# mathwrx/Decouple-and-Couple_Learning_in_Multi-Modal_Brain_Tumor_Segmentation

Hardware: AMD Instinct MI355X
Metric: training volumes/sec (4x128^3) (higher is better)
Workload: dtype bf16x3 forward (split-bf16 MFMA operands hi.hi+hi.lo+lo.hi: logits within 1e-3 of the fp32 reference) / bf16 data-gradient / bf16 weight-gradient MFMA operands; f32 accumulate, f32 storage, f32 master weights; 1 GPU; configs[1]: 1xMI355X, batch 2 per GPU, 4-modality 128^3 synthetic BraTS patches; fwd + softmax_dice + 4 sub-region/edge losses + bwd + Adam(amsgrad); random-init weights, dropout on; global_batch=2, parallelism=dp1, precision=bf16x3, dgrad_precision=bf16, wgrad_precision=bf16, mode=plan

## Files before the change

decouple-and-couple_learning_in_multi-modal_brain_tumor_segmentation_amd/csrc/conv_args.h:

```cpp
#pragma once
#include "common.h"

typedef __bf16 bf16x8 __attribute__((ext_vector_type(8)));
typedef unsigned u32x4 __attribute__((ext_vector_type(4)));

struct ConvArgsB {
  ConvGeom g;
  const float* x; const uint4* wpk; const float* bias; float* y;
  const float* in_scale; const float* in_shift; float in_slope;
  const float* residual; int r_ldc; const float* out_scale; double* stats;
  unsigned long long unused_[2];
  const float* nb_x; int nb_ldc; const float* nb_scale; const float* nb_shift; float nb_slope;
  int groups, x_goff, y_goff;
  const uint4* wpk_g[3]; const float* bias_g[3];
  const uint4* x16; const uint4* zero16;
  unsigned short* y16;
};

typedef __bf16 bf16x2_t __attribute__((ext_vector_type(2)));
typedef float f32x2_t __attribute__((ext_vector_type(2)));
__device__ __forceinline__ unsigned pack_bf16(float a, float b) {
  const f32x2_t f = {a, b};
  return __builtin_bit_cast(unsigned, __builtin_convertvector(f, bf16x2_t));
}
__device__ __forceinline__ float bf16_round(float a) { return (float)(__bf16)a; }
__device__ __forceinline__ void split_bf16(float a, float b, unsigned& hi, unsigned& lo) {
  hi = pack_bf16(a, b);
  const float ha = __builtin_bit_cast(float, hi << 16), hb = __builtin_bit_cast(float, hi & 0xffff0000u);
  lo = pack_bf16(a - ha, b - hb);
}
__device__ __forceinline__ float act01(float v, float slope) { return fmaxf(v, v * slope); }


static inline int cfg_extent(int op, int Di, int Hi, int Wi, int Do, int Ho, int Wo, int cd[3]) {
  cd[0] = Do; cd[1] = Ho; cd[2] = Wo;
  if (op == CWF_CONVT2) { cd[0] = Di; cd[1] = Hi; cd[2] = Wi; return 8; }
  if (op == CWF_CONV3_S2_DGRAD) { cd[0] = (Do + 1) / 2; cd[1] = (Ho + 1) / 2; cd[2] = (Wo + 1) / 2; return 8; }
  return 1;
}

int cwf_try_conv_ws(int op, int x3, ConvArgsB& a, hipStream_t st, int* rc);
int cwf_ws_takes_x16(int op, int N, int D, int H, int W, int Cin, int Cout);
int cwf_ws_takes_x3();
int cwf_try_conv_wsp(int op, int x3, int cfg_mt, int cfg_wm, ConvArgsB& a, hipStream_t st, int* rc);
int cwf_try_conv_wsd(int op, int x3, int cfg_mt, int cfg_wm, ConvArgsB& a, hipStream_t st, int* rc);

int conv_fp32_launch(const cwf_conv_args& d, hipStream_t st);
int conv_stem_launch(const cwf_conv_args& d, hipStream_t st);
int conv_s2c16_launch(const cwf_conv_args& d, hipStream_t st);
int wgrad_fp32_launch(const cwf_wgrad_args& d, int* nsplit_used, hipStream_t st);
```

decouple-and-couple_learning_in_multi-modal_brain_tumor_segmentation_amd/csrc/conv_bf16.hip:

```cpp
#include "common.h"
#include <cstdio>
#include <cstdlib>
#include <type_traits>

#include "conv_args.h"

#define CB_MAXS 13
struct StageSlots { int goff[CB_MAXS]; unsigned inb; int nslots; };

__device__ __forceinline__ void stage_slots_init(StageSlots& ss, const ConvGeom& g, int id0, int ih0, int iw0, int tid) {
  const int nvox_in = g.ID * g.IH * g.IW;
  ss.nslots = (nvox_in + 63) >> 6; ss.inb = 0u;
  const int dq = 64 / g.IW, dr = 64 - dq * g.IW;
  int iw = (tid >> 2) % g.IW, t2 = (tid >> 2) / g.IW;
  int ih = t2 % g.IH, idd = t2 / g.IH;
#pragma unroll
  for (int i = 0; i < CB_MAXS; ++i) {
    const int v = (tid >> 2) + 64 * i;
    const int gd = id0 + idd, gh = ih0 + ih, gw = iw0 + iw;
    const bool ok = v < nvox_in && gd >= 0 && gd < g.Di && gh >= 0 && gh < g.Hi && gw >= 0 && gw < g.Wi;
    ss.goff[i] = ok ? ((gd * g.Hi + gh) * g.Wi + gw) * g.x_ldc : 0;
    ss.inb |= ok ? (1u << i) : 0u;
    iw += dr; int adv = dq;
    if (iw >= g.IW) { iw -= g.IW; ++adv; }
// ... 1149 lines not shown
    }
    if (d.y16) return CWF_E_BADARG;
  }
  {
    int rcw = 0;
    if (cwf_try_conv_wsp(op, x3, c.MT, c.WM, a, st, &rcw)) return rcw;
    if (cwf_try_conv_wsd(op, x3, c.MT, c.WM, a, st, &rcw)) return rcw;
    if (cwf_try_conv_ws(op, x3, a, st, &rcw)) return rcw;
  }
  if (op == CWF_CONV3_S1 && Cin <= 16 && Cout <= 16) c16_tap_order(a.g);
  if (op == CWF_CONV3_S1 && Cin <= 16 && Cout <= 16 && (int64_t)d.Do * d.Ho * d.Wo >= 32768) {
    rc = cwf_build_geom(a.g, op, N, d.Di, d.Hi, d.Wi, Cin, x_ldc, d.Do, d.Ho, d.Wo, Cout, y_ldc, 16);
    if (rc) return rc;
    return x3 ? launch_conv16s<true>(a, st) : launch_conv16s<false>(a, st);
  }
#define CWF_CFG(mt, nt, wm) if (c.MT == mt && c.NT == nt && c.WM == wm) return x3 ? launch_cfg<mt, nt, wm, true>(a, st) : launch_cfg<mt, nt, wm, false>(a, st);
  CWF_CFG(4, 4, 1) CWF_CFG(2, 4, 2) CWF_CFG(2, 4, 4) CWF_CFG(4, 2, 4) CWF_CFG(4, 1, 4)
  CWF_CFG(1, 4, 4) CWF_CFG(1, 2, 4) CWF_CFG(1, 2, 2) CWF_CFG(1, 1, 4)
#undef CWF_CFG
  return CWF_E_BADARG;
}

static int conv_grouped_impl(const cwf_conv_args& d, hipStream_t st) {
  const int op = d.op, x3 = d.precision == CWF_BF16X3, groups = d.groups, N = d.N, Cin = d.Cin, Cout = d.Cout;
  const int x_ldc = d.x_ldc, y_ldc = d.y_ldc, x_goff = d.x_goff, y_goff = d.y_goff;
  if (!d.x || !d.y || N <= 0 || Cin <= 0 || Cout <= 0) return CWF_E_BADARG;
  if ((Cin & 3) || (x_ldc & 3) || (x_goff & 3) || x_ldc < (groups - 1) * x_goff + Cin || y_ldc < (groups - 1) * y_goff + Cout) return CWF_E_ALIGN;
  if ((uintptr_t)d.x & 15) return CWF_E_ALIGN;
  ConvArgsB a;
  int cd[3];
  TileCfg c = choose_cfg(op, cd, cfg_extent(op, d.Di, d.Hi, d.Wi, d.Do, d.Ho, d.Wo, cd), N * groups, cdiv(Cout, 16));
  int rc = cwf_build_geom(a.g, op, N, d.Di, d.Hi, d.Wi, Cin, x_ldc, d.Do, d.Ho, d.Wo, Cout, y_ldc, c.MT * c.WM);
  if (rc) return rc;
  a.x = d.x; a.wpk = nullptr; a.bias = nullptr; a.y = d.y; a.in_scale = nullptr; a.in_shift = nullptr; a.in_slope = 1.f;
  a.residual = nullptr; a.r_ldc = 0; a.out_scale = nullptr; a.stats = nullptr;
  a.nb_x = nullptr; a.nb_ldc = 0; a.nb_scale = nullptr; a.nb_shift = nullptr; a.nb_slope = 1.f;
  a.groups = groups; a.x_goff = x_goff; a.y_goff = y_goff;
  a.x16 = nullptr; a.zero16 = nullptr; a.y16 = nullptr;
  for (int q = 0; q < 3; ++q) {
    a.wpk_g[q] = q < groups ? reinterpret_cast<const uint4*>(d.wpk_g[q]) : nullptr;
    a.bias_g[q] = q < groups ? d.bias_g[q] : nullptr;
    if (q < groups && (!d.wpk_g[q] || ((uintptr_t)d.wpk_g[q] & 15))) return CWF_E_ALIGN;
  }
  if (Cin <= 16 && Cout <= 16) c16_tap_order(a.g);
#define CWF_CFG(mt, nt, wm) if (c.MT == mt && c.NT == nt && c.WM == wm) return x3 ? launch_cfg<mt, nt, wm, true>(a, st) : launch_cfg<mt, nt, wm, false>(a, st);
  CWF_CFG(4, 4, 1) CWF_CFG(2, 4, 2) CWF_CFG(2, 4, 4) CWF_CFG(4, 2, 4) CWF_CFG(4, 1, 4)
  CWF_CFG(1, 4, 4) CWF_CFG(1, 2, 4) CWF_CFG(1, 2, 2) CWF_CFG(1, 1, 4)
#undef CWF_CFG
  return CWF_E_BADARG;
}

extern "C" int cwf_conv_x16_ok(int op, int N, int D, int H, int W, int Cin, int Cout) {
  if (op != CWF_CONV3_S1 || N <= 0 || D <= 0 || H <= 0 || W <= 0) return 0;
  if (Cin == 16 && Cout == 16) return (int64_t)D * H * W >= 32768 && (int64_t)N * D * H * W < (1ll << 30);
  return cwf_ws_takes_x16(op, N, D, H, W, Cin, Cout);
}

extern "C" int cwf_conv(const struct cwf_conv_args* args, void* stream) {
  if (!args) return CWF_E_BADARG;
  const cwf_conv_args& d = *args;
  if (d.precision != CWF_FP32 && d.precision != CWF_BF16X3 && d.precision != CWF_BF16) return CWF_E_BADARG;
  const bool fp32 = d.precision == CWF_FP32;
  hipStream_t st = cwf_stream(stream);
  if (d.groups) {
    if (d.groups < 2 || d.groups > 3 || d.op != CWF_CONV3_S1 || d.in_scale || d.residual || d.out_scale || d.stats || d.nb_x || d.x16 ||
        d.y16 || d.w_raw)
      return CWF_E_BADARG;
    if (!fp32) return conv_grouped_impl(d, st);
    for (int q = 0; q < d.groups; ++q) {
      cwf_conv_args g = d;
      g.groups = 0; g.x = d.x + q * d.x_goff; g.y = d.y + q * d.y_goff; g.wpk = d.wpk_g[q]; g.bias = d.bias_g[q];
      const int rc = conv_fp32_launch(g, st);
      if (rc) return rc;
    }
    return 0;
  }
  if (d.x16) {
    if (d.precision != CWF_BF16 || d.in_scale || d.out_scale || d.y16 || !d.zero16 || ((uintptr_t)d.x16 & 15) || ((uintptr_t)d.zero16 & 15))
      return CWF_E_BADARG;
    if (d.Do != d.Di || d.Ho != d.Hi || d.Wo != d.Wi || !cwf_conv_x16_ok(d.op, d.N, d.Di, d.Hi, d.Wi, d.Cin, d.Cout))
      return CWF_E_BADARG;
    return conv_bf16_impl(d, st);
  }
  if (d.y16) {
    if (d.nb_x || d.out_scale) return CWF_E_BADARG;
    if (!fp32 && d.op == CWF_CONV1) {
      const int rc = conv_bf16_impl(d, st);
      if (rc != CWF_E_BADARG) return rc;
    }
    cwf_conv_args f = d;
    f.y16 = nullptr;
    const int rc = cwf_conv(&f, stream);
    if (rc) return rc;
    return cwf_to_bf16(d.y, d.y_ldc, nullptr, nullptr, 1.f, d.y16, d.N, (int64_t)d.Do * d.Ho * d.Wo, d.Cout, stream);
  }
  const int64_t vo = (int64_t)d.Do * d.Ho * d.Wo;
  if (d.w_raw && !fp32 && !d.in_scale && !d.residual && !d.nb_x) {
    if (d.op == CWF_CONV3_S1 && d.Cin == 4 && d.Cout == 16 && vo >= 32768) return conv_stem_launch(d, st);
    if (d.op == CWF_CONV3_S2 && d.Cin == 16 && d.Cout == 32 && !d.out_scale && vo >= 32768 &&
        d.Do == (d.Di + 1) / 2 && d.Ho == (d.Hi + 1) / 2 && d.Wo == (d.Wi + 1) / 2)
      return conv_s2c16_launch(d, st);
  }
  if (fp32) return d.nb_x ? CWF_E_BADARG : conv_fp32_launch(d, st);
  return conv_bf16_impl(d, st);
}
```

decouple-and-couple_learning_in_multi-modal_brain_tumor_segmentation_amd/cwf/_lib.py:

```python
from __future__ import annotations

import ctypes as C
import os

_HERE = os.path.dirname(os.path.abspath(__file__))
LIB_PATH = os.path.join(_HERE, "libcwf_hip.so")

P = C.c_void_p
I = C.c_int
L = C.c_int64
F = C.c_float
U = C.c_uint32
U64 = C.c_uint64
D = C.c_double

SIGNATURES = {
    "cwf_version": [],
    "cwf_conv": [P, P],
    "cwf_conv_x16_ok": [I, I, I, I, I, I, I],
    "cwf_debug_wsd": [I],
    "cwf_debug_wsd_launches": [],
    "cwf_wgrad": [P, P, P],
    "cwf_debug_wgrad_bf16_plan": [P, P],
    "cwf_debug_wgrad_bf16_name": [I],
    "cwf_debug_wgrad_s2": [I],
    "cwf_debug_wgrad_s2_launches": [],
    "cwf_gather_split_bf16": [P, I, L, P],
    "cwf_wgrad_nsplit": [I, I, I, I, I, I, I],
    "cwf_wgrad_partial_floats": [I, I, I, I, I, I, I],
    "cwf_wgrad_slab_floats": [I, I, I],
    "cwf_wgrad_reduce": [P, I, L, P, P, P, P],
    "cwf_gather_batched": [P, I, L, P],
    "cwf_in_finalize": [P, P, P, I, L, F, P],
    "cwf_in_stats": [P, I, P, I, L, I, P],
    "cwf_norm_act_add": [P, I, P, P, F, P, I, P, I, I, L, I, P],
    "cwf_in_bwd_stats": [P, I, P, I, P, P, F, P, I, L, I, P],
    "cwf_in_bwd_apply": [P, I, P, I, P, P, F, P, P, I, P, I, I, L, I, P],
    "cwf_in_bwd_apply_ex": [P, I, P, I, P, P, F, P, P, I, P, I, P, P, I, L, I, P],
    "cwf_norm_act_add_ex": [P, I, P, P, F, P, I, P, I, P, I, L, I, P],
    "cwf_to_bf16": [P, I, P, P, F, P, I, L, I, P],
    "cwf_gemm": [P, L, L, L, L, P, L, L, L, L, P, L, L, L, P, P, L, L, L, I, I, I, I, I, F, I, I, P],
    "cwf_layernorm_fwd": [P, P, P, P, P, P, I, I, F, P],
    "cwf_layernorm_bwd": [P, P, P, P, P, P, P, P, I, I, I, P],
    "cwf_softmax_rows": [P, L, I, I, P],
    "cwf_softmax_rows_bwd": [P, P, L, I, I, P],
    "cwf_gelu_bwd": [P, P, P, L, P],
    "cwf_colsum": [P, L, I, I, P, I, P],
    "cwf_window_to_tokens": [P, I, P, I, I, I, I, I, I, I, I, P],
    "cwf_tokens_to_window": [P, P, I, I, I, I, I, I, I, I, I, I, P],
    "cwf_token_scores": [P, P, L, P, I, I, I, P],
    "cwf_topk": [P, P, I, I, I, P],
    "cwf_gather_tokens": [P, P, P, L, P, F, P, I, I, I, I, P],
    "cwf_gather_tokens_bwd": [P, P, P, P, P, L, I, I, I, I, P],
    "cwf_scatter_rows": [P, P, P, L, L, P, L, P, I, I, I, I, P],
    "cwf_scatter_rows_bwd": [P, P, P, P, L, P, I, P, L, L, P, L, I, I, I, I, P],
    "cwf_upsample_softmax": [P, I, P, I, I, I, I, I, I, P],
    "cwf_upsample_softmax_bwd": [P, P, P, I, I, I, I, I, I, I, P, P],
    "cwf_channel_softmax": [P, I, P, L, I, P],
    "cwf_channel_softmax_bwd": [P, P, P, I, L, I, P],
    "cwf_dice_ce_sums": [P, P, U, P, I, L, I, P],
    "cwf_dice_ce_finalize": [P, P, P, I, L, I, P],
    "cwf_dice_ce_bwd": [P, P, U, P, P, P, I, L, I, P],
    "cwf_adam_amsgrad": [P, I, L, C.c_double, C.c_double, C.c_double, C.c_double, C.c_double, I, I, P, P],
    "cwf_adam_amsgrad_scaled": [P, I, L, C.c_double, C.c_double, C.c_double, C.c_double, C.c_double, I, I, P, F, P],
    "cwf_grad_add": [P, P, P, L, P],
    "cwf_grad_norm_clip": [P, L, F, F, P, P, P],
    "cwf_adam_amsgrad_ex": [P, I, L, C.c_double, C.c_double, C.c_double, C.c_double, C.c_double, I, I, P, F, P, P, F, P],
    "cwf_optim_step": [I, P, I, L, C.c_double, C.c_double, P, C.c_double, C.c_double, C.c_double, I, I, P, C.c_double, C.c_double, I, I,
                       F, P, P, F, P],
    "cwf_wgrad_reduce_batched": [P, I, P],
    "cwf_dropout_mask": [P, L, F, F, C.c_uint64, C.c_uint64, P],
    "cwf_mul": [P, P, P, L, P],
    "cwf_add": [P, P, P, L, P],
    "cwf_channel_scale": [P, I, P, P, I, I, L, I, P],
    "cwf_copy_strided": [P, I, P, I, L, I, P],
    "cwf_add3": [P, P, P, P, L, P],
    "cwf_bcast3": [P, P, L, P],
    "cwf_stats_channel_sum": [P, P, I, I, P],
    "cwf_gemm_ex": [P, P],
    "cwf_debug_gemm_panel": [I],
    "cwf_debug_gemm_panel_launches": [],
    "cwf_attn_fwd": [P, L, P, L, I, I, I, I, F, P, U64, F, P],
    "cwf_attn_bwd": [P, L, P, L, P, I, I, I, I, F, P, U64, F, P],
    "cwf_attn_bwd_ws": [P, L, P, L, P, I, I, I, I, F, P, U64, F, P, L, P],
    "cwf_attn_bwd_ws_bytes": [I, I, I],
    "cwf_debug_attn_split": [I],
    "cwf_debug_attn_split_waves": [I],
    "cwf_debug_attn_split_launches": [],
    "cwf_ln_pair_fwd": [P, P, I, P, P, P, P, P, P, P, I, I, F, P],
    "cwf_ln_pair_bwd": [P, P, P, P, P, I, P, P, P, P, P, P, P, P, P, I, I, I, P],
    "cwf_gelu_bwd_drop": [P, P, P, L, P, U64, F, P],
    "cwf_token_scores2": [P, P, L, P, L, P, P, I, I, I, P],
    "cwf_topk_inv": [P, P, P, P, P, P, I, I, I, P],
    "cwf_index_inv": [P, P, I, I, I, P],
    "cwf_gather_multi": [P, I, I, I, I, F, P, F, P],
    "cwf_scatter_inv": [P, P, P, L, L, P, L, P, P, I, I, I, P],
    "cwf_scatter_bwd": [P, P, P, P, P, P, L, L, P, L, P, L, P, L, L, P, L, I, I, I, I, P],
    "cwf_debug_scatter_bwd": [I],
    "cwf_token_grad": [P, P, P, L, P, P, P, L, P, L, P, U64, U64, F, P, I, I, I, I, P],
    "cwf_head_grad": [P, P, P, P, L, P, P, I, I, P],
    "cwf_dice_ce_finalize_multi": [P, P, P, P, I, I, L, I, P],
    "cwf_head_loss_sums": [P, I, I, P, P, P, I, I, I, I, I, P],
    "cwf_head_loss_bwd": [P, I, I, P, P, P, P, P, I, P, I, I, I, I, I, P],
    "cwf_head_loss_bwd_ex": [P, I, I, P, P, P, P, P, I, I, P, I, I, I, I, I, P],
# ... 114 lines not shown

class WgradArgs(C.Structure):
    _fields_ = [("op", I), ("precision", I),
                ("x", P), ("x_ldc", I), ("in_scale", P), ("in_shift", P), ("in_slope", F),
                ("dy", P), ("dy_ldc", I),
                ("dy_scale", P), ("xa16", P), ("dy16", P), ("zero16", P),
                ("partial", P),
                ("groups", I), ("x_g", P * 3), ("dy_g", P * 3), ("partial_g", P * 3),
                ("N", I), ("Di", I), ("Hi", I), ("Wi", I), ("Cin", I), ("Do", I), ("Ho", I), ("Wo", I), ("Cout", I)]


PRECISION = {"fp32": 0, "bf16x3": 1, "bf16": 2}


class LnGroupParams(C.Structure):
    _fields_ = [(n, P * 4) for n in ("g1", "b1", "g2", "b2", "dg1", "db1", "dg2", "db2")]


class GatherJob(C.Structure):
    _fields_ = [("feats", P), ("index", P), ("head", P), ("out", P), ("head_bstride", L), ("out_bstride", L), ("T", I),
                ("drop_off", C.c_uint64), ("head_g", P * 4), ("group_B", I)]


class PrepSample(C.Structure):
    _fields_ = [("image", P), ("label", P), ("S0", I), ("S1", I), ("S2", I), ("o0", I), ("o1", I), ("o2", I), ("flip", I),
                ("intensity", I), ("scale", F * 4), ("shift", F * 4)]


class PrepAffineSample(C.Structure):
    _fields_ = PrepSample._fields_ + [("m", F * 9)]


class PrepElasticSample(C.Structure):
    _fields_ = PrepAffineSample._fields_ + [("disp", P), ("G0", I), ("G1", I), ("G2", I)]


class IntensitySample(C.Structure):
    _fields_ = [("taps", (F * 7) * 4), ("amp", F * 4), ("key", U64), ("gamma", F * 4), ("blur", I), ("noise", I), ("gam", I)]


class FocalParams(C.Structure):
    _fields_ = [("fn", D), ("fp", D), ("exponent", D), ("smooth", D), ("gamma", D), ("ce_ratio", D), ("class_weight", D * 4)]


INTENSITY_TILE = (10, 10, 32)


def intensity_ws_floats(nb, crop):
    tiles = 1
    for c, t in zip(crop, INTENSITY_TILE):
        tiles *= (int(c) + t - 1) // t
    return 8 * int(nb) * tiles


class AcquireSample(C.Structure):
    _fields_ = [("bias", P * 4), ("G0", I), ("G1", I), ("G2", I), ("bias_mask", I), ("contrast_mask", I), ("lowres_mask", I),
                ("factor", F * 4), ("lattice", (I * 3) * 4)]


ACQUIRE_TILE = (32, 8, 32)


def acquire_ws_doubles(nb, crop):
    tiles = 1
    for c, t in zip(crop, ACQUIRE_TILE):
        tiles *= (int(c) + t - 1) // t
    return 12 * int(nb) * tiles


WINDOW_MAX_STARTS = 128


class WindowGrid(C.Structure):
    _fields_ = [("B", I), ("S", I * 3), ("r", I * 3), ("n", I * 3), ("start", (I * WINDOW_MAX_STARTS) * 3)]


class WindowBox(C.Structure):
    _fields_ = [("full", I * 3), ("lo", I * 3)]


NORM_WS_DOUBLES = 2568
GRADNORM_WS_DOUBLES = 1024
RULE_ADAMW, RULE_SGD = 1, 2
RESTYPE_INT64 = {"cwf_debug_wsd_launches", "cwf_debug_wgrad_s2_launches", "cwf_debug_gemm_panel_launches", "cwf_debug_attn_split_launches", "cwf_attn_bwd_ws_bytes", "cwf_wgrad_partial_floats", "cwf_wgrad_slab_floats", "cwf_hausdorff_workspace", "cwf_components_workspace",
                 "cwf_lesionwise_workspace", "cwf_surface_metrics_workspace", "cwf_lesionwise_ex_workspace", "cwf_signed_distance_workspace",
                 "cwf_topk_ce_workspace", "cwf_focal_workspace", "cwf_lovasz_workspace", "cwf_class_locations_workspace", "cwf_nonzero_box_workspace"}
LOCATIONS_TILE = 16384
NONZERO_BOX_TILE = 4096

_lib = None


class CwfError(RuntimeError):
    pass


def load():
    global _lib
    if _lib is not None:
        return _lib
    if not os.path.exists(LIB_PATH):
        raise CwfError("libcwf_hip.so is not built (%s); run `python __graft_entry__.py` or `make -C csrc`. "
                       "There is no CPU fallback." % LIB_PATH)
    lib = C.CDLL(LIB_PATH)
    for name, args in SIGNATURES.items():
        fn = getattr(lib, name)
        fn.argtypes = args
        fn.restype = L if name in RESTYPE_INT64 else I
    lib.cwf_arch.restype = C.c_char_p
    lib.cwf_arch.argtypes = []
    lib.cwf_plan_last_error.restype = C.c_char_p
    lib.cwf_plan_last_error.argtypes = []
    lib.cwf_debug_wgrad_bf16_name.restype = C.c_char_p
    _lib = lib
    return lib


def check(rc, name):
    if rc != 0:
        raise CwfError("%s failed with status %d" % (name, rc))
```

include/cwf_hip.h:

```cpp
#ifndef CWF_HIP_H
#define CWF_HIP_H
#include <stdint.h>
#ifdef __cplusplus
extern "C" {
#endif

#define CWF_E_BADARG   (-1)
#define CWF_E_TOOLARGE (-2)
#define CWF_E_ALIGN    (-3)

int cwf_version(void);
const char* cwf_arch(void);

enum { CWF_CONV3_S1 = 0, CWF_CONV3_S2 = 1, CWF_CONV1 = 2, CWF_CONVT2 = 3, CWF_CONV3_S2_DGRAD = 4, CWF_CONVT2_DGRAD = 5 };
enum { CWF_FP32 = 0, CWF_BF16X3 = 1, CWF_BF16 = 2 };

struct cwf_conv_args {
  int op, precision;
  const float* x; int x_ldc; const void* wpk; const float* bias; float* y; int y_ldc;
  const float* in_scale; const float* in_shift; float in_slope;
  const float* residual; int r_ldc; const float* out_scale; double* stats;
  const float* nb_x; int nb_ldc; const float* nb_scale; const float* nb_shift; float nb_slope;
  const void* x16; const void* zero16; void* y16;
  const float* w_raw;
  int groups, x_goff, y_goff; const void* wpk_g[3]; const float* bias_g[3];
  int N, Di, Hi, Wi, Cin, Do, Ho, Wo, Cout;
};
int cwf_conv(const struct cwf_conv_args* args , void* stream);
int cwf_conv_x16_ok(int op, int N, int D, int H, int W, int Cin, int Cout);
int cwf_debug_wsd(int v);
long long cwf_debug_wsd_launches(void);

int cwf_wgrad_nsplit(int op, int N, int Do, int Ho, int Wo, int Cin, int Cout);
int64_t cwf_wgrad_partial_floats(int op, int N, int Do, int Ho, int Wo, int Cin, int Cout);
int64_t cwf_wgrad_slab_floats(int op, int Cin, int Cout);
struct cwf_wgrad_args {
  int op, precision;
  const float* x; int x_ldc; const float* in_scale; const float* in_shift; float in_slope;
  const float* dy; int dy_ldc;
  const float* dy_scale; const void* xa16; const void* dy16; const void* zero16;
  float* partial;
  int groups; const float* x_g[3]; const float* dy_g[3]; float* partial_g[3];
  int N, Di, Hi, Wi, Cin, Do, Ho, Wo, Cout;
};
int cwf_wgrad(const struct cwf_wgrad_args* args , int* nsplit_used , void* stream);
enum cwf_wgrad_bf16_instance {
  CWF_WGB_WGRAD16 = 0, CWF_WGB_WGRAD16_X3,
  CWF_WGB_PW_1_1_1, CWF_WGB_PW_2_1_1, CWF_WGB_PW_4_2_1, CWF_WGB_PW_8_4_1,
  CWF_WGB_PW_1_1_8, CWF_WGB_PW_2_2_8,
  CWF_WGB_S1_1, CWF_WGB_S1_2,
  CWF_WGB_TILED_7_1, CWF_WGB_TILED_7_1_X3, CWF_WGB_TILED_7_2, CWF_WGB_TILED_7_2_X3,
  CWF_WGB_TILED_2_1, CWF_WGB_TILED_2_1_X3, CWF_WGB_TILED_2_2, CWF_WGB_TILED_2_2_X3,
  CWF_WGB_TILED_2_4, CWF_WGB_TILED_2_4_X3,
  CWF_WGB_WGRAD16D, CWF_WGB_S1D,
  CWF_WGB_COUNT
};
enum { CWF_WGB_WALK_RANGES = 0, CWF_WGB_WALK_STRIDED = 1, CWF_WGB_WALK_PW = 2 };
#define CWF_WGB_PLAN_FIELDS 15
int cwf_debug_wgrad_bf16_plan(const struct cwf_wgrad_args* args , int64_t* out );
const char* cwf_debug_wgrad_bf16_name(int instance);
int cwf_debug_wgrad_s2(int v);
long long cwf_debug_wgrad_s2_launches(void);
int cwf_wgrad_reduce(const float* partial, int nsplit, int64_t slab_floats,
                     const int32_t* inv_map, float* dW, float* db, void* stream);
struct cwf_wgrad_reduce_desc { const float* partial; const int32_t* inv; float* dW; float* db; int64_t slab; int32_t nsplit; int32_t pad_; };
int cwf_wgrad_reduce_batched(const struct cwf_wgrad_reduce_desc* table, int nlayers, void* stream);

struct cwf_gather_desc { const float* src; float* dst; const int32_t* map; int64_t n; };

int cwf_gather_split_bf16(const struct cwf_gather_desc* table, int nlayers, int64_t max_n, void* stream);

int cwf_gather_batched(const struct cwf_gather_desc* table, int nlayers, int64_t max_n, void* stream);

int cwf_in_finalize(const double* stats, float* scale, float* shift, int NC, int64_t V, float eps, void* stream);
int cwf_in_stats(const float* x, int x_ldc, double* stats, int N, int64_t V, int C, void* stream);
int cwf_norm_act_add(const float* x, int x_ldc, const float* scale, const float* shift, float slope,
                     const float* residual, int r_ldc, float* y, int y_ldc, int N, int64_t V, int C, void* stream);
int cwf_in_bwd_stats(const float* dy, int dy_ldc, const float* x, int x_ldc, const float* scale, const float* shift,
                     float slope, double* sums, int N, int64_t V, int C, void* stream);
int cwf_in_bwd_apply(const float* dy, int dy_ldc, const float* x, int x_ldc, const float* scale, const float* shift,
                     float slope, const double* sums, const float* dx_add, int a_ldc, float* dx, int dx_ldc,
                     int N, int64_t V, int C, void* stream);

int cwf_in_bwd_apply_ex(const float* dy, int dy_ldc, const float* x, int x_ldc, const float* scale, const float* shift,
                        float slope, const double* sums, const float* dx_add, int a_ldc, float* dx, int dx_ldc,
                        void* dx16, void* xa16, int N, int64_t V, int C, void* stream);
int cwf_norm_act_add_ex(const float* x, int x_ldc, const float* scale, const float* shift, float slope,
                        const float* residual, int r_ldc, float* y, int y_ldc, void* y16, int N, int64_t V, int C, void* stream);
int cwf_to_bf16(const float* x, int x_ldc, const float* scale, const float* shift, float slope, void* y16,
                int N, int64_t V, int C, void* stream);
int cwf_gemm(const float* A, int64_t sa_m, int64_t sa_k, int64_t sa_zb, int64_t sa_zh,
             const float* B, int64_t sb_k, int64_t sb_n, int64_t sb_zb, int64_t sb_zh,
             float* C, int64_t sc_m, int64_t sc_zb, int64_t sc_zh,
             const float* bias, const float* residual, int64_t sr_m, int64_t sr_zb, int64_t sr_zh,
             int M, int Nn, int K, int ZB, int ZH, float alpha, int act, int accumulate, void* stream);
struct cwf_gemm_args {
  const float* A; int64_t sa_m, sa_k, sa_zb, sa_zh;
  const float* B; int64_t sb_k, sb_n, sb_zb, sb_zh;
  float* C; int64_t sc_m, sc_zb, sc_zh;
  const float* bias; const float* residual; int64_t sr_m, sr_zb, sr_zh;
  int M, N, K, ZB, ZH; float alpha; int act; int accumulate;
  const float* A2; int split_n;
  const float* B2; int split_m;
  float* C2;
  float* rowsum; int rowsum_acc;
  const uint64_t* rng;
  uint64_t a_drop_off, a_drop_n; float a_drop_p, a_drop_p2;
  uint64_t c_drop_off, c_drop_n; float c_drop_p, c_drop_p2;
  const float* B_tab[4]; const float* bias_tab[4]; float* C_tab[4]; float* rowsum_tab[4];
};
int cwf_gemm_ex(const struct cwf_gemm_args* args , void* stream);
int cwf_debug_gemm_panel(int v);
long long cwf_debug_gemm_panel_launches(void);

// ... 321 lines not shown
```

Baseline: 123.0 volumes/s.

## Add dedicated bf16 MFMA kernel for stride-2 conv data-gradient

Adds a new persistent kernel for the stride-2 3x3x3 conv data-gradient in bf16. It stages input halos into double-buffered LDS, prefetches the next tile while computing the current one, and decomposes output parity classes into 14 MFMA steps per channel chunk. Residual add and an optional bf16 output copy are fused into the epilogue. It is dispatched for four channel shapes when the output volume is large enough, replacing the generic path. In exchange it adds a large specialized code path with its own weight packing assumptions.

```diff
diff --git a/decouple-and-couple_learning_in_multi-modal_brain_tumor_segmentation_amd/csrc/conv_args.h b/decouple-and-couple_learning_in_multi-modal_brain_tumor_segmentation_amd/csrc/conv_args.h
--- a/decouple-and-couple_learning_in_multi-modal_brain_tumor_segmentation_amd/csrc/conv_args.h
+++ b/decouple-and-couple_learning_in_multi-modal_brain_tumor_segmentation_amd/csrc/conv_args.h
@@ -44,6 +44,7 @@
 int cwf_ws_takes_x3();
 int cwf_try_conv_wsp(int op, int x3, int cfg_mt, int cfg_wm, ConvArgsB& a, hipStream_t st, int* rc);
 int cwf_try_conv_wsd(int op, int x3, int cfg_mt, int cfg_wm, ConvArgsB& a, hipStream_t st, int* rc);
+int cwf_try_conv_s2d(const cwf_conv_args& d, hipStream_t st, int* rc);
 
 int conv_fp32_launch(const cwf_conv_args& d, hipStream_t st);
 int conv_stem_launch(const cwf_conv_args& d, hipStream_t st);
diff --git a/decouple-and-couple_learning_in_multi-modal_brain_tumor_segmentation_amd/csrc/conv_bf16.hip b/decouple-and-couple_learning_in_multi-modal_brain_tumor_segmentation_amd/csrc/conv_bf16.hip
--- a/decouple-and-couple_learning_in_multi-modal_brain_tumor_segmentation_amd/csrc/conv_bf16.hip
+++ b/decouple-and-couple_learning_in_multi-modal_brain_tumor_segmentation_amd/csrc/conv_bf16.hip
@@ -1255,6 +1255,10 @@
       return CWF_E_BADARG;
     return conv_bf16_impl(d, st);
   }
+  if (d.op == CWF_CONV3_S2_DGRAD && d.precision == CWF_BF16) {
+    int rcs = 0;
+    if (cwf_try_conv_s2d(d, st, &rcs)) return rcs;
+  }
   if (d.y16) {
     if (d.nb_x || d.out_scale) return CWF_E_BADARG;
     if (!fp32 && d.op == CWF_CONV1) {
diff --git a/decouple-and-couple_learning_in_multi-modal_brain_tumor_segmentation_amd/csrc/conv_s2d.hip b/decouple-and-couple_learning_in_multi-modal_brain_tumor_segmentation_amd/csrc/conv_s2d.hip
--- /dev/null
+++ b/decouple-and-couple_learning_in_multi-modal_brain_tumor_segmentation_amd/csrc/conv_s2d.hip
@@ -0,0 +1,365 @@
+#include "common.h"
+#include <type_traits>
+
+#include "conv_args.h"
+
+namespace {
+
+constexpr int S2D_HV = 3 * 3 * 17;
+
+__host__ __device__ constexpr int s2d_e_cls(int e) { constexpr int t[14] = {0, 1, 2, 3, 3, 4, 5, 5, 6, 6, 7, 7, 7, 7}; return t[e]; }
+__host__ __device__ constexpr int s2d_e_step(int e) { constexpr int t[14] = {0, 0, 0, 0, 1, 0, 0, 1, 0, 1, 0, 1, 2, 3}; return t[e]; }
+__host__ __device__ constexpr int s2d_e_frag(int e) { constexpr int t[14] = {0, 1, 2, 1, 3, 4, 1, 5, 2, 6, 1, 3, 5, 7}; return t[e]; }
+__host__ __device__ constexpr int s2d_cls_pairs(int c) { constexpr int t[8] = {1, 1, 1, 2, 1, 2, 2, 4}; return t[c]; }
+__host__ __device__ constexpr int s2d_cls_pre(int c) { constexpr int t[8] = {0, 1, 2, 3, 5, 6, 8, 10}; return t[c]; }
+template <int NCH, int NT>
+__host__ __device__ constexpr int s2d_blk(int chunk, int e, int j) {
+  return ((s2d_cls_pre(s2d_e_cls(e)) * NCH + chunk * s2d_cls_pairs(s2d_e_cls(e)) + s2d_e_step(e)) * NT + j);
+}
+
+struct S2dArgs {
+  const float* x; const uint4* wpk; float* y; const float* residual; unsigned short* y16;
+  int x_ldc, y_ldc, r_ldc;
+  int N, Di, Hi, Wi, Do, Ho, Wo;
+  int tiles_d, tiles_h, tiles_w, total_tiles, tiles_per_wg;
+};
+
+template <int NCH, int NT, bool WLDS>
+__global__ __launch_bounds__(256, (NT == 1 ? 3 : NT == 2 ? 2 : 1)) void conv_s2d_kernel(const S2dArgs a) {
+  constexpr int GPV = NCH * 4;
+  constexpr int VS = 256 / GPV;
+  constexpr int SLOTS = (S2D_HV + VS - 1) / VS;
+  constexpr int SG = 5;
+  constexpr int NGRP = SLOTS / SG;
+  constexpr int CPG = NCH / NGRP;
+  static_assert(SLOTS % SG == 0 && NCH % NGRP == 0, "staging groups");
+  constexpr int IMG = NCH * S2D_HV * 16;
+  constexpr int NBLK = NCH * 14 * NT;
+  constexpr int TOT = NCH * 14;
+  constexpr int PD = NT == 4 ? 2 : 4;
+  extern __shared__ float4 lds4[];
+  unsigned short* img = reinterpret_cast<unsigned short*>(lds4);
+  uint4* wlds = reinterpret_cast<uint4*>(img + 2 * IMG);
+
+  const int tid = threadIdx.x, lane = tid & 63;
+  const int wave = __builtin_amdgcn_readfirstlane(tid >> 6);
+  const int r = lane & 15, kq = lane >> 4;
+  const bool second = (kq >> 1) != 0;
+  const int td = wave >> 1, th = wave & 1;
+
+  int bx = blockIdx.x;
+  {
+    const int nb = gridDim.x;
+    if ((nb & 7) == 0) bx = (bx & 7) * (nb >> 3) + (bx >> 3);
+  }
+  const int t_begin = bx * a.tiles_per_wg;
+  const int t_end = min(a.total_tiles, t_begin + a.tiles_per_wg);
+  if (t_begin >= t_end) return;
+
+  if (WLDS) {
+    for (int i = tid; i < NBLK * 64; i += 256) wlds[i] = a.wpk[(i >> 6) * 128 + (i & 63) * 2];
+  }
+  const unsigned wl_off = (unsigned)lane * 32u;
+
+  const int sq = tid % GPV, v0 = tid / GPV;
+  const int ldo0 = ((sq >> 2) * S2D_HV + v0) * 16 + (sq & 3) * 4;
+  int rel[SLOTS], pos[SLOTS];
+#pragma unroll
+  for (int i = 0; i < SLOTS; ++i) {
+    const int v = v0 + i * VS;
+    const bool live = v < S2D_HV;
+    const int vc = live ? v : 0;
+    const int vw = vc % 17, vh = (vc / 17) % 3, vd = vc / 51;
+    rel[i] = ((vd * a.Hi + vh) * a.Wi + vw) * a.x_ldc + sq * 4;
+    pos[i] = live ? (vd | (vh << 2) | (vw << 4)) : (3 | (3 << 2) | (31 << 4));
+  }
+
+  struct Tile { int n, d0, h0, w0; };
+  auto tile_of = [&](int t) __attribute__((always_inline)) {
+    Tile tl;
+    const int tw = t % a.tiles_w; t /= a.tiles_w;
+    const int thh = t % a.tiles_h; t /= a.tiles_h;
+    const int tdd = t % a.tiles_d;
+    tl.n = t / a.tiles_d; tl.d0 = tdd * 2; tl.h0 = thh * 2; tl.w0 = tw * 16;
+    return tl;
+  };
+
+  float4 val[SG]; unsigned okm = 0u;
+  auto issue = [&](auto GRP_, const Tile& tl) __attribute__((always_inline)) {
+    constexpr int GRP = decltype(GRP_)::value;
+    const float* xb = a.x + ((((int64_t)tl.n * a.Di + tl.d0) * a.Hi + tl.h0) * a.Wi + tl.w0) * a.x_ldc;
+    const int rd = a.Di - tl.d0, rh = a.Hi - tl.h0, rw = a.Wi - tl.w0;
+    okm = 0u;
+#pragma unroll
+    for (int k = 0; k < SG; ++k) {
+      const int i = GRP * SG + k;
+      int ps = pos[i]; asm volatile("" : "+v"(ps));
+      const bool ok = (ps & 3) < rd && ((ps >> 2) & 3) < rh && (ps >> 4) < rw;
+      okm |= ok ? (1u << k) : 0u;
+      val[k] = *reinterpret_cast<const float4*>(xb + (ok ? rel[i] : 0));
+    }
+  };
+  auto commit = [&](auto GRP_, unsigned short* ib) __attribute__((always_inline)) {
+    constexpr int GRP = decltype(GRP_)::value;
+#pragma unroll
+    for (int k = 0; k < SG; ++k) {
+      const int i = GRP * SG + k;
+      const bool ok = (okm >> k) & 1u;
+      uint2 h;
+      h.x = pack_bf16(val[k].x, val[k].y); h.y = pack_bf16(val[k].z, val[k].w);
+      h.x = ok ? h.x : 0u; h.y = ok ? h.y : 0u;
+      if (v0 + i * VS < S2D_HV) *reinterpret_cast<uint2*>(ib + ldo0 + i * VS * 16) = h;
+    }
+  };
+
+  const int ab = ((td * 3 + th) * 17 + r) * 16 + (kq & 1) * 8;
+  const int b0 = ab, bw = ab + (second ? 16 : 0), bh = ab + (second ? 17 * 16 : 0), bd = ab + (second ? 51 * 16 : 0);
+
+  int vx[2][4];
+#pragma unroll
+  for (int i = 0; i < 4; ++i) {
+    vx[0][i] = NT == 1 ? 2 * ((kq & ~1) * 4 + i) + (kq & 1) : 2 * (kq * 4 + i);
+    vx[1][i] = vx[0][i] + (NT == 1 ? 8 : 1);
+  }
+  const bool kodd = (kq & 1) != 0;
+
+  auto do_tile = [&](int t, int buf, auto PF_) __attribute__((always_inline)) {
+    constexpr bool PF = decltype(PF_)::value;
+    const Tile tl = tile_of(t);
+    const Tile nx = tile_of(PF ? t + 1 : t);
+    const unsigned short* ib = img + buf * IMG;
+    unsigned short* ob = img + (buf ^ 1) * IMG;
+    uint4 ring[PD][NT];
+    auto load_b = [&](int S, int slot) __attribute__((always_inline)) {
+#pragma unroll
+      for (int j = 0; j < NT; ++j) {
+        if (WLDS) { ring[slot][j] = wlds[s2d_blk<NCH, NT>(S / 14, S % 14, j) * 64 + lane]; continue; }
+        unsigned bo = wl_off; asm volatile("" : "+v"(bo));
+        ring[slot][j] = *reinterpret_cast<const uint4*>(reinterpret_cast<const char*>(a.wpk) + (bo + (unsigned)(s2d_blk<NCH, NT>(S / 14, S % 14, j) * 2048)));
+      }
+    };
+    if (!WLDS) {
+#pragma unroll
+      for (int d = 0; d < PD; ++d) load_b(d, d);
+    }
+    __syncthreads();
+    if (PF) issue(std::integral_constant<int, 0>{}, nx);
+    if (WLDS) {
+#pragma unroll
+      for (int d = 0; d < PD; ++d) load_b(d, d);
+    }
+
+    f32x4 acc[8][NT];
+#pragma unroll
+    for (int c = 0; c < 8; ++c)
+#pragma unroll
+      for (int j = 0; j < NT; ++j) acc[c][j] = (f32x4){0.f, 0.f, 0.f, 0.f};
+    auto chunks = [&](auto G_) __attribute__((always_inline)) {
+      constexpr int G = decltype(G_)::value;
+#pragma unroll
+      for (int chunk = G * CPG; chunk < (G + 1) * CPG; ++chunk) {
+        const unsigned short* icp = ib + chunk * S2D_HV * 16;
+        uint4 fr[8];
+        fr[0] = *reinterpret_cast<const uint4*>(icp + b0);
+        fr[1] = *reinterpret_cast<const uint4*>(icp + bw);
+        fr[2] = *reinterpret_cast<const uint4*>(icp + bh);
+        fr[3] = *reinterpret_cast<const uint4*>(icp + bw + 17 * 16);
+        fr[4] = *reinterpret_cast<const uint4*>(icp + bd);
+        fr[5] = *reinterpret_cast<const uint4*>(icp + bw + 51 * 16);
+        fr[6] = *reinterpret_cast<const uint4*>(icp + bh + 51 * 16);
+        fr[7] = *reinterpret_cast<const uint4*>(icp + bw + 68 * 16);
+#pragma unroll
+        for (int e = 0; e < 14; ++e) {
+          const int S = chunk * 14 + e;
+          uint4 b[NT];
+#pragma unroll
+          for (int j = 0; j < NT; ++j) b[j] = ring[S % PD][j];
+          if (S + PD < TOT) load_b(S + PD, S % PD);
+#pragma unroll
+          for (int j = 0; j < NT; ++j)
+            acc[s2d_e_cls(e)][j] = __builtin_amdgcn_mfma_f32_16x16x32_bf16(__builtin_bit_cast(bf16x8, fr[s2d_e_frag(e)]),
+                                                                           __builtin_bit_cast(bf16x8, b[j]), acc[s2d_e_cls(e)][j], 0, 0, 0);
+          __builtin_amdgcn_sched_barrier(0);
+        }
+      }
+    };
+    chunks(std::integral_constant<int, 0>{});
+    if constexpr (NGRP >= 2) {
+      if (PF) { commit(std::integral_constant<int, 0>{}, ob); issue(std::integral_constant<int, 1>{}, nx); }
+      chunks(std::integral_constant<int, 1>{});
+    }
+    if constexpr (NGRP >= 4) {
+      if (PF) { commit(std::integral_constant<int, 1>{}, ob); issue(std::integral_constant<int, 2>{}, nx); }
+      chunks(std::integral_constant<int, 2>{});
+      if (PF) { commit(std::integral_constant<int, 2>{}, ob); issue(std::integral_constant<int, 3>{}, nx); }
+      chunks(std::integral_constant<int, 3>{});
+    }
+
+    const int jd = tl.d0 + td, jh = tl.h0 + th;
+    const bool full = 2 * jd + 1 < a.Do && 2 * jh + 1 < a.Ho && 2 * (tl.w0 + 16) <= a.Wo;
+    auto epi = [&](auto FULL_, auto RES_, auto IMG_) __attribute__((always_inline)) {
+      constexpr bool FULL = decltype(FULL_)::value, RES = decltype(RES_)::value, IMG16 = decltype(IMG_)::value;
+      constexpr int GB = NT == 1 ? 4 : 1;
+      const int wleft = a.Wo - 2 * tl.w0;
+      unsigned yo[2][4], ro[2][4], io[2][4];
+#pragma unroll
+      for (int h = 0; h < 2; ++h)
+#pragma unroll
+        for (int i = 0; i < 4; ++i) {
+          yo[h][i] = (unsigned)(vx[h][i] * a.y_ldc + r) * 4u; asm volatile("" : "+v"(yo[h][i]));
+          if (RES) { ro[h][i] = (unsigned)(vx[h][i] * a.r_ldc + r) * 4u; asm volatile("" : "+v"(ro[h][i])); }
+          if (IMG16) { io[h][i] = (unsigned)(vx[h][i] * (NT * 16) + r) * 2u; asm volatile("" : "+v"(io[h][i])); }
+        }
+#pragma unroll
+      for (int g0 = 0; g0 < 4; g0 += GB) {
+        float rv[GB][2][NT][4];
+        if (RES) {
+#pragma unroll
+          for (int gg = 0; gg < GB; ++gg) {
+            const int g = g0 + gg, od = 2 * jd + (g >> 1), oh = 2 * jh + (g & 1);
+            const bool rowok = od < a.Do && oh < a.Ho;
+            const int64_t vox0 = (((int64_t)tl.n * a.Do + od) * a.Ho + oh) * a.Wo + 2 * tl.w0;
+            const char* rb = reinterpret_cast<const char*>(a.residual + vox0 * a.r_ldc);
+#pragma unroll
+            for (int h = 0; h < 2; ++h)
+#pragma unroll
+              for (int j = 0; j < NT; ++j)
+#pragma unroll
+                for (int i = 0; i < 4; ++i) {
+                  rv[gg][h][j][i] = 0.f;
+                  if (FULL || (rowok && vx[h][i] < wleft)) rv[gg][h][j][i] = *reinterpret_cast<const float*>(rb + ro[h][i] + j * 64);
+                }
+          }
+        }
+#pragma unroll
+        for (int gg = 0; gg < GB; ++gg) {
+          const int g = g0 + gg, od = 2 * jd + (g >> 1), oh = 2 * jh + (g & 1);
+          const bool rowok = od < a.Do && oh < a.Ho;
+          const int64_t vox0 = (((int64_t)tl.n * a.Do + od) * a.Ho + oh) * a.Wo + 2 * tl.w0;
+          char* yb = reinterpret_cast<char*>(a.y + vox0 * a.y_ldc);
+          char* ib16 = IMG16 ? reinterpret_cast<char*>(a.y16 + vox0 * (NT * 16)) : nullptr;
+#pragma unroll
+          for (int j = 0; j < NT; ++j)
+#pragma unroll
+            for (int i = 0; i < 4; ++i) {
+              const float ev = acc[2 * g][j][i], ov = acc[2 * g + 1][j][i];
+              float o[2];
+              if (NT == 1) {
+                const float got = __shfl_xor(kodd ? ev : ov, 16, 64);
+                o[0] = kodd ? got : ev; o[1] = kodd ? ov : got;
+              } else { o[0] = ev; o[1] = ov; }
+#pragma unroll
+              for (int h = 0; h < 2; ++h) {
+                float v = o[h] + 0.f;
+                if (RES) v += rv[gg][h][j][i];
+                if (FULL || (rowok && vx[h][i] < wleft)) {
+                  *reinterpret_cast<float*>(yb + yo[h][i] + j * 64) = v;
+                  if (IMG16) *reinterpret_cast<unsigned short*>(ib16 + io[h][i] + j * 32) = (unsigned short)(pack_bf16(v, v) & 0xffffu);
+                }
+              }
+            }
+        }
+      }
+    };
+    using T_ = std::true_type; using F_ = std::false_type;
+    if (jd < a.Di && jh < a.Hi) {
+      if (a.y16) {
+        if (full) { if (a.residual) epi(T_{}, T_{}, T_{}); else epi(T_{}, F_{}, T_{}); }
+        else      { if (a.residual) epi(F_{}, T_{}, T_{}); else epi(F_{}, F_{}, T_{}); }
+      } else {
+        if (full) { if (a.residual) epi(T_{}, T_{}, F_{}); else epi(T_{}, F_{}, F_{}); }
+        else      { if (a.residual) epi(F_{}, T_{}, F_{}); else epi(F_{}, F_{}, F_{}); }
+      }
+    }
+    if (PF) commit(std::integral_constant<int, NGRP - 1>{}, ob);
+  };
+
+  {
+    const Tile tl = tile_of(t_begin);
+    issue(std::integral_constant<int, 0>{}, tl); commit(std::integral_constant<int, 0>{}, img);
+    if constexpr (NGRP >= 2) { issue(std::integral_constant<int, 1>{}, tl); commit(std::integral_constant<int, 1>{}, img); }
+    if constexpr (NGRP >= 4) {
+      issue(std::integral_constant<int, 2>{}, tl); commit(std::integral_constant<int, 2>{}, img);
+      issue(std::integral_constant<int, 3>{}, tl); commit(std::integral_constant<int, 3>{}, img);
+    }
+  }
+  int buf = 0;
+#pragma unroll 1
+  for (int t = t_begin; t < t_end - 1; ++t) { do_tile(t, buf, std::true_type{}); buf ^= 1; }
+  do_tile(t_end - 1, buf, std::false_type{});
+}
+
+int s2d_grid(int total_tiles, int nch, int nt, int* tiles_per_wg) {
+  const bool wlds = nch == 2;
+  const int per_cu = wlds ? (nt == 1 ? 3 : 2) : (nt == 4 ? 1 : 2);
+  int grid = 256 * per_cu; if (grid > total_tiles) grid = total_tiles;
+  *tiles_per_wg = cdiv(total_tiles, grid);
+  return cdiv(total_tiles, *tiles_per_wg);
+}
+
+template <int NCH, int NT, bool WLDS>
+int s2d_launch(S2dArgs& a, hipStream_t st) {
+  const size_t lds = (size_t)2 * NCH * S2D_HV * 16 * sizeof(unsigned short) + (WLDS ? (size_t)NCH * 14 * NT * 1024 : 0);
+  const int grid = s2d_grid(a.total_tiles, NCH, NT, &a.tiles_per_wg);
+  CWF_MAX_LDS_ONCE((&conv_s2d_kernel<NCH, NT, WLDS>));
+  hipLaunchKernelGGL((conv_s2d_kernel<NCH, NT, WLDS>), dim3(grid), dim3(256), lds, st, a);
+  CWF_LAUNCH_CHECK();
+  return 0;
+}
+
+int g_s2d = 1;
+long long g_s2d_launches = 0;
+
+bool s2d_shape_ok(int op, int precision, int N, int Do, int Ho, int Wo, int Cin, int Cout) {
+  if (!g_s2d || op != CWF_CONV3_S2_DGRAD || precision != CWF_BF16 || N <= 0 || Do <= 0 || Ho <= 0 || Wo <= 0) return false;
+  if (!((Cin == 32 && Cout == 16) || (Cin == 64 && Cout == 32) || (Cin == 32 && Cout == 32) || (Cin == 128 && Cout == 64))) return false;
+  if (g_s2d == 1 && (int64_t)Do * Ho * Wo < 32768) return false;
+  return true;
+}
+
+}
+
+extern "C" int cwf_debug_s2d(int v) { const int old = g_s2d; g_s2d = v; return old; }
+extern "C" long long cwf_debug_s2d_launches() { return g_s2d_launches; }
+
+extern "C" int cwf_conv_y16_fused_ok(int op, int precision, int N, int Do, int Ho, int Wo, int Cin, int Cout) {
+  if (!s2d_shape_ok(op, precision, N, Do, Ho, Wo, Cin, Cout)) return 0;
+  return (int64_t)N * Do * Ho * Wo * Cout * 4 < (1ll << 31);
+}
+
+int cwf_try_conv_s2d(const cwf_conv_args& d, hipStream_t st, int* rc) {
+  if (!s2d_shape_ok(d.op, d.precision, d.N, d.Do, d.Ho, d.Wo, d.Cin, d.Cout)) return 0;
+  if (d.in_scale || d.in_shift || d.in_slope != 1.f || d.bias || d.out_scale || d.stats || d.nb_x || d.groups || d.x16 || d.w_raw) return 0;
+  if (!d.x || !d.wpk || !d.y) return 0;
+  if (d.Di != (d.Do + 1) / 2 || d.Hi != (d.Ho + 1) / 2 || d.Wi != (d.Wo + 1) / 2) return 0;
+  if ((d.x_ldc & 3) || d.x_ldc < d.Cin || d.y_ldc < d.Cout || ((uintptr_t)d.x & 15) || ((uintptr_t)d.wpk & 15)) return 0;
+  if (d.residual && d.r_ldc < d.Cout) return 0;
+  if (d.y16 && ((uintptr_t)d.y16 & 1)) return 0;
+  const int64_t vo = (int64_t)d.N * d.Do * d.Ho * d.Wo, vi = (int64_t)d.N * d.Di * d.Hi * d.Wi;
+  const int64_t ld = d.residual && d.r_ldc > d.y_ldc ? d.r_ldc : d.y_ldc;
+  if (vo * ld * 4 >= (1ll << 31) || vi * d.x_ldc * 4 >= (1ll << 31)) return 0;
+  S2dArgs a;
+  a.x = d.x; a.wpk = reinterpret_cast<const uint4*>(d.wpk); a.y = d.y; a.residual = d.residual;
+  a.y16 = reinterpret_cast<unsigned short*>(d.y16);
+  a.x_ldc = d.x_ldc; a.y_ldc = d.y_ldc; a.r_ldc = d.r_ldc;
+  a.N = d.N; a.Di = d.Di; a.Hi = d.Hi; a.Wi = d.Wi; a.Do = d.Do; a.Ho = d.Ho; a.Wo = d.Wo;
+  a.tiles_d = cdiv(d.Di, 2); a.tiles_h = cdiv(d.Hi, 2); a.tiles_w = cdiv(d.Wi, 16);
+  a.total_tiles = d.N * a.tiles_d * a.tiles_h * a.tiles_w;
+  a.tiles_per_wg = 1;
+  if (d.Cin == 32 && d.Cout == 16) *rc = s2d_launch<2, 1, true>(a, st);
+  else if (d.Cin == 32 && d.Cout == 32) *rc = s2d_launch<2, 2, true>(a, st);
+  else if (d.Cin == 64 && d.Cout == 32) *rc = s2d_launch<4, 2, false>(a, st);
+  else *rc = s2d_launch<8, 4, false>(a, st);
+  if (*rc == 0) ++g_s2d_launches;
+  return 1;
+}
+
+extern "C" int cwf_debug_s2d_plan(int N, int Do, int Ho, int Wo, int Cin, int Cout, int* out) {
+  if (!out || !s2d_shape_ok(CWF_CONV3_S2_DGRAD, CWF_BF16, N, Do, Ho, Wo, Cin, Cout)) return 0;
+  const int Di = (Do + 1) / 2, Hi = (Ho + 1) / 2, Wi = (Wo + 1) / 2;
+  const int per_sample = cdiv(Di, 2) * cdiv(Hi, 2) * cdiv(Wi, 16), total = N * per_sample;
+  int tpw = 1;
+  const int grid = s2d_grid(total, Cin / 16, Cout / 16, &tpw);
+  out[0] = total; out[1] = grid; out[2] = tpw; out[3] = per_sample;
+  return 1;
+}
diff --git a/decouple-and-couple_learning_in_multi-modal_brain_tumor_segmentation_amd/cwf/_lib.py b/decouple-and-couple_learning_in_multi-modal_brain_tumor_segmentation_amd/cwf/_lib.py
--- a/decouple-and-couple_learning_in_multi-modal_brain_tumor_segmentation_amd/cwf/_lib.py
+++ b/decouple-and-couple_learning_in_multi-modal_brain_tumor_segmentation_amd/cwf/_lib.py
@@ -20,6 +20,10 @@
     "cwf_conv_x16_ok": [I, I, I, I, I, I, I],
     "cwf_debug_wsd": [I],
     "cwf_debug_wsd_launches": [],
+    "cwf_debug_s2d": [I],
+    "cwf_debug_s2d_launches": [],
+    "cwf_conv_y16_fused_ok": [I, I, I, I, I, I, I, I],
+    "cwf_debug_s2d_plan": [I, I, I, I, I, I, P],
     "cwf_wgrad": [P, P, P],
     "cwf_debug_wgrad_bf16_plan": [P, P],
     "cwf_debug_wgrad_bf16_name": [I],
@@ -300,7 +304,7 @@
 NORM_WS_DOUBLES = 2568
 GRADNORM_WS_DOUBLES = 1024
 RULE_ADAMW, RULE_SGD = 1, 2
-RESTYPE_INT64 = {"cwf_debug_wsd_launches", "cwf_debug_wgrad_s2_launches", "cwf_debug_gemm_panel_launches", "cwf_debug_attn_split_launches", "cwf_attn_bwd_ws_bytes", "cwf_wgrad_partial_floats", "cwf_wgrad_slab_floats", "cwf_hausdorff_workspace", "cwf_components_workspace",
+RESTYPE_INT64 = {"cwf_debug_wsd_launches", "cwf_debug_s2d_launches","cwf_debug_wgrad_s2_launches", "cwf_debug_gemm_panel_launches", "cwf_debug_attn_split_launches", "cwf_attn_bwd_ws_bytes", "cwf_wgrad_partial_floats", "cwf_wgrad_slab_floats", "cwf_hausdorff_workspace", "cwf_components_workspace",
                  "cwf_lesionwise_workspace", "cwf_surface_metrics_workspace", "cwf_lesionwise_ex_workspace", "cwf_signed_distance_workspace",
                  "cwf_topk_ce_workspace", "cwf_focal_workspace", "cwf_lovasz_workspace", "cwf_class_locations_workspace", "cwf_nonzero_box_workspace"}
 LOCATIONS_TILE = 16384
diff --git a/include/cwf_hip.h b/include/cwf_hip.h
--- a/include/cwf_hip.h
+++ b/include/cwf_hip.h
@@ -30,6 +30,10 @@
 int cwf_conv_x16_ok(int op, int N, int D, int H, int W, int Cin, int Cout);
 int cwf_debug_wsd(int v);
 long long cwf_debug_wsd_launches(void);
+int cwf_debug_s2d(int v);
+long long cwf_debug_s2d_launches(void);
+int cwf_conv_y16_fused_ok(int op, int precision, int N, int Do, int Ho, int Wo, int Cin, int Cout);
+int cwf_debug_s2d_plan(int N, int Do, int Ho, int Wo, int Cin, int Cout, int* out);
 
 int cwf_wgrad_nsplit(int op, int N, int Do, int Ho, int Wo, int Cin, int Cout);
 int64_t cwf_wgrad_partial_floats(int op, int N, int Do, int Ho, int Wo, int Cin, int Cout);
```

Result: no change. 123.8 volumes/s, median of 6 (+0.6%).
